# Rose-STL-Lab/spherical-dyffusion

Hardware: AMD Instinct MI355X
Metric: forecast-steps/sec (180x360, 63ch), 25-member ensemble DYffusion sampling, whole job (higher is better)
Workload: dtype f32 tensors; every GEMM-class kernel (1x1 convs, fused MLP, Legendre analysis/synthesis, dhconv) as 3-pass split-f16 MFMA with f32 accumulation; FFT / norms / pointwise in f32 (statistics f64)

## Files before the change

### include/sdy_amd.h

```cpp
#ifndef SDY_AMD_H
#define SDY_AMD_H

#include <stddef.h>
#include <stdint.h>

#ifdef __cplusplus
extern "C" {
#endif
#pragma GCC visibility push(default)

#define SDY_OK 0
#define SDY_ERR_ARG (-1)
#define SDY_ERR_UNSUPPORTED (-2)
#define SDY_ERR_ALIGN (-3)
#define SDY_ERR_WORKSPACE (-4)
#define SDY_ERR_NAME (-5)
#define SDY_ERR_SHAPE (-6)
#define SDY_ERR_STATE (-7)

#define SDY_GRID_EQUIANGULAR 0
#define SDY_GRID_LEGENDRE_GAUSS 1

int sdy_version(void);
const char* sdy_error_string(int code);
// ... 30 lines not shown
int sdy_gelu_stats(const float* y, long y_bstride, float* out, long out_bstride, int out_tiled, double* stats, int B, int C,
                   int HW, void* stream);
int sdy_affine_copy_stats(const float* x, long x_bstride, const float* a, const float* d, float* out, long out_bstride,
                          double* stats, int C, int HW, const unsigned char* rows, int n_rows, int src_row0, void* stream);

int sdy_dhconv_pack_weight(const float* w_host, int Ci, int Co, int L, float* w_packed_dev, void* stream);
int sdy_dhconv(const float* Cs_in, const float* w_packed, float* Cs_out, int L, int mtr, int B, int Ci, int Co,
               void* stream);
size_t sdy_dhconv_h3_pack_bytes(int Ci, int Co, int L);
int sdy_dhconv_h3_pack_weight(const float* w_host, int Ci, int Co, int L, void* packed_dev, float* scale);
int sdy_dhconv_h3(const float* Cs_in, const void* packed, float scale, float* Cs_out, int L, int mtr, int B, int Ci,
                  int Co, void* stream);

int sdy_dhconv_frag_supported(int Ci, int Co);
size_t sdy_dhconv_frag_pack_bytes(int L);
int sdy_dhconv_frag_pack(const float* w_host, int L, void* packed_dev, float* scale);
int sdy_dhconv_frag(const float* Cs_in, const void* packed, float scale, float* Cs_out, int L, int mtr, int B,
                    void* stream);

int sdy_instnorm_coeffs(const float* x, int B, int C, int HW, const float* gamma, const float* beta,
                        const float* scale_shift, long ss_stride, float eps, float* a, float* d, void* stream);

typedef struct sdy_conv_args {
  const float* x;  long x_bstride;
  const float* wt; int ldw;
  float* out;      long out_bstride;
  int B, Cin, Cout, HW;
  const float* pa; const float* pd;
  const float* bias;
  const float* add; long add_bstride;
  int add_mode;
  int act;
  float drop_p;
  const float* keep_mask;
  uint64_t seed; uint32_t call; uint32_t stream_id; uint32_t batch_offset;
  int rows_per_call;
  const float* batch_scale;
  int kernel_tag;
  const void* w_h3;
  float w_h3_scale;
  const void* w_frag;
  float w_frag_scale;
  double* stats;
  int out_tiled;
  const unsigned char* x_rows;
} sdy_conv_args;
int sdy_conv1x1(const sdy_conv_args* args, void* stream);

int sdy_conv256_h3_supported(int Cin, int Cout);
size_t sdy_conv256_h3_pack_bytes(void);
size_t sdy_conv256_h3_pack_bytes_cin(int Cin);
int sdy_conv256_h3_pack(const float* w_host, void* packed_dev, float* scale);
int sdy_conv256_h3_pack_cin(const float* w_host, int Cin, void* packed_dev, float* scale);
size_t sdy_h3_pack_bytes(int Cout, int Cin);
int sdy_h3_pack_weight(const float* w_host, int Cout, int Cin, void* packed_dev, float* scale);

typedef struct sdy_mlp_args {
  const float* x;  long x_bstride;
  const float* pa; const float* pd;
  const void* w; float w1_scale; float w2_scale;
  const float* b1; const float* b2;
  float* out;      long out_bstride;
  const float* add; long add_bstride;
  const float* add_a; const float* add_d;
  int B, E, hidden, HW;
  float drop_p;
  uint64_t seed; uint32_t call; uint32_t stream_fc1; uint32_t stream_fc2; uint32_t batch_offset;
  int rows_per_call;
  const float* batch_scale;
  double* stats;
  int x_tiled;
  const float* keep_hidden;
  const float* keep_out;
  const unsigned char* out_rows;
  int add_by_launch_row;
} sdy_mlp_args;
int sdy_instnorm_from_stats(double* stats, int B, int C, int HW, const float* gamma, const float* beta,
                            const float* scale_shift, long ss_bstride, float eps, float* a_out, float* d_out, void* stream);
int sdy_mlp_h3_supported(int E, int hidden);
size_t sdy_mlp_h3_pack_bytes(int E, int hidden);
int sdy_mlp_h3_pack(const float* w1_host, const float* w2_host, int E, int hidden, void* packed_dev, float* scale1,
                    float* scale2);
int sdy_mlp_h3(const sdy_mlp_args* args, void* stream);

typedef struct sdy_pair_args {
  const float* x;  long x_bstride;
  const void* w; float w1_scale; float w2_scale;
  const float* b1;
  float* out;      long out_bstride;
  const float* add; long add_bstride;
  int B, Cin, hidden, Cout, HW;
  double* stats;
} sdy_pair_args;
int sdy_pair_h3_supported(int Cin, int hidden, int Cout);
size_t sdy_pair_h3_pack_bytes(int Cin, int hidden, int Cout);
int sdy_pair_h3_pack(const float* w1_host, const float* w2_host, int Cin, int hidden, int Cout, void* packed_dev,
                     float* scale1, float* scale2);
int sdy_pair_h3(const sdy_pair_args* args, void* stream);

typedef struct sdy_sfno_config {
  int nlat, nlon;
  int in_chans;
  int out_chans;
  int embed_dim;
  int num_layers;
  int mlp_hidden;
// ... 594 lines not shown
```

### spherical-dyffusion_amd/_lib.py

```python
from __future__ import annotations

import ctypes as C
import os

_HERE = os.path.dirname(os.path.abspath(__file__))
LIB_PATH = os.environ.get("SDY_AMD_LIB") or os.path.join(_HERE, "libsdy_amd.so")

SDY_GRID = {"equiangular": 0, "legendre-gauss": 1}


class SdyError(RuntimeError):
    pass


class SdyConvArgs(C.Structure):
    _fields_ = [
        ("x", C.c_void_p), ("x_bstride", C.c_long),
        ("wt", C.c_void_p), ("ldw", C.c_int),
        ("out", C.c_void_p), ("out_bstride", C.c_long),
        ("B", C.c_int), ("Cin", C.c_int), ("Cout", C.c_int), ("HW", C.c_int),
        ("pa", C.c_void_p), ("pd", C.c_void_p),
        ("bias", C.c_void_p),
        ("add", C.c_void_p), ("add_bstride", C.c_long),
        ("add_mode", C.c_int),
# ... 556 lines not shown
    "sdy_sht_tables_host": (C.c_int, [C.c_int, C.c_int, C.c_int, C.c_int, C.c_int, C.c_void_p, C.c_void_p, C.c_void_p]),
    "sdy_sht_plan_create": (C.c_int, [C.c_int, C.c_int, C.c_int, C.c_int, C.c_int, C.POINTER(C.c_void_p)]),
    "sdy_sht_plan_create_ex": (C.c_int, [C.c_int, C.c_int, C.c_int, C.c_int, C.c_int, C.c_int, C.POINTER(C.c_void_p)]),
    "sdy_sht_plan_destroy": (None, [C.c_void_p]),
    "sdy_sht_plan_dims": (C.c_int, [C.c_void_p, C.POINTER(C.c_int * 6)]),
    "sdy_sht_plan_kernels": (C.c_int, [C.c_void_p, C.POINTER(C.c_int * 2)]),
    "sdy_sht_workspace_floats": (C.c_size_t, [C.c_void_p, C.c_int, C.c_int]),
    "sdy_sht_forward": (C.c_int, [C.c_void_p, C.c_void_p, C.c_void_p, C.c_int, C.c_int, C.c_void_p, C.c_size_t, C.c_void_p]),
    "sdy_sht_inverse": (C.c_int, [C.c_void_p, C.c_void_p, C.c_void_p, C.c_int, C.c_int, C.c_void_p, C.c_size_t, C.c_void_p]),
    "sdy_rfft_lon": (C.c_int, [C.c_void_p, C.c_void_p, C.c_void_p, C.c_void_p, C.c_void_p, C.c_void_p, C.c_int, C.c_int, C.c_void_p]),
    "sdy_legendre_fwd": (C.c_int, [C.c_void_p, C.c_void_p, C.c_void_p, C.c_int, C.c_int, C.c_void_p]),
    "sdy_legendre_inv": (C.c_int, [C.c_void_p, C.c_void_p, C.c_void_p, C.c_int, C.c_int, C.c_void_p]),
    "sdy_irfft_lon": (C.c_int, [C.c_void_p, C.c_void_p, C.c_void_p, C.c_void_p, C.c_int, C.c_int, C.c_void_p]),
    "sdy_irfft_lon_act": (C.c_int, [C.c_void_p, C.c_void_p, C.c_void_p, C.c_void_p, C.c_long, C.c_void_p, C.c_int, C.c_int,
                                    C.c_void_p]),
    "sdy_instnorm_from_partials": (C.c_int, [C.c_void_p, C.c_int, C.c_int, C.c_int, C.c_int, C.c_void_p, C.c_void_p, C.c_float,
                                             C.c_void_p, C.c_void_p, C.c_void_p]),
    "sdy_gelu_stats": (C.c_int, [C.c_void_p, C.c_long, C.c_void_p, C.c_long, C.c_int, C.c_void_p, C.c_int, C.c_int, C.c_int,
                                 C.c_void_p]),
    "sdy_affine_copy_stats": (C.c_int, [C.c_void_p, C.c_long, C.c_void_p, C.c_void_p, C.c_void_p, C.c_long, C.c_void_p, C.c_int,
                                        C.c_int, C.c_void_p, C.c_int, C.c_int, C.c_void_p]),
    "sdy_dhconv_pack_weight": (C.c_int, [C.c_void_p, C.c_int, C.c_int, C.c_int, C.c_void_p, C.c_void_p]),
    "sdy_dhconv": (C.c_int, [C.c_void_p, C.c_void_p, C.c_void_p, C.c_int, C.c_int, C.c_int, C.c_int, C.c_int, C.c_void_p]),
    "sdy_dhconv_h3_pack_bytes": (C.c_size_t, [C.c_int, C.c_int, C.c_int]),
    "sdy_dhconv_h3_pack_weight": (C.c_int, [C.c_void_p, C.c_int, C.c_int, C.c_int, C.c_void_p, C.POINTER(C.c_float)]),
    "sdy_dhconv_h3": (C.c_int, [C.c_void_p, C.c_void_p, C.c_float, C.c_void_p, C.c_int, C.c_int, C.c_int, C.c_int, C.c_int,
                                C.c_void_p]),
    "sdy_dhconv_frag_supported": (C.c_int, [C.c_int, C.c_int]),
    "sdy_dhconv_frag_pack_bytes": (C.c_size_t, [C.c_int]),
    "sdy_dhconv_frag_pack": (C.c_int, [C.c_void_p, C.c_int, C.c_void_p, C.POINTER(C.c_float)]),
    "sdy_dhconv_frag": (C.c_int, [C.c_void_p, C.c_void_p, C.c_float, C.c_void_p, C.c_int, C.c_int, C.c_int, C.c_void_p]),
    "sdy_instnorm_coeffs": (C.c_int, [C.c_void_p, C.c_int, C.c_int, C.c_int, C.c_void_p, C.c_void_p, C.c_void_p, C.c_long,
                                      C.c_float, C.c_void_p, C.c_void_p, C.c_void_p]),
    "sdy_conv1x1": (C.c_int, [C.POINTER(SdyConvArgs), C.c_void_p]),
    "sdy_ensemble_metrics": (C.c_int, [C.c_void_p, C.c_void_p, C.c_void_p, C.c_int, C.c_long, C.c_int, C.c_int, C.c_void_p,
                                       C.c_void_p]),
    "sdy_instnorm_from_stats": (C.c_int, [C.c_void_p, C.c_int, C.c_int, C.c_int, C.c_void_p, C.c_void_p, C.c_void_p,
                                          C.c_long, C.c_float, C.c_void_p, C.c_void_p, C.c_void_p]),
    "sdy_mlp_h3_supported": (C.c_int, [C.c_int, C.c_int]),
    "sdy_mlp_h3_pack_bytes": (C.c_size_t, [C.c_int, C.c_int]),
    "sdy_mlp_h3_pack": (C.c_int, [C.c_void_p, C.c_void_p, C.c_int, C.c_int, C.c_void_p, C.POINTER(C.c_float),
                                  C.POINTER(C.c_float)]),
    "sdy_mlp_h3": (C.c_int, [C.POINTER(SdyMlpArgs), C.c_void_p]),
    "sdy_pair_h3_supported": (C.c_int, [C.c_int, C.c_int, C.c_int]),
    "sdy_pair_h3_pack_bytes": (C.c_size_t, [C.c_int, C.c_int, C.c_int]),
    "sdy_pair_h3_pack": (C.c_int, [C.c_void_p, C.c_void_p, C.c_int, C.c_int, C.c_int, C.c_void_p, C.POINTER(C.c_float),
                                   C.POINTER(C.c_float)]),
    "sdy_pair_h3": (C.c_int, [C.POINTER(SdyPairArgs), C.c_void_p]),
    "sdy_conv256_h3_supported": (C.c_int, [C.c_int, C.c_int]),
    "sdy_conv256_h3_pack_bytes": (C.c_size_t, []),
    "sdy_conv256_h3_pack_bytes_cin": (C.c_size_t, [C.c_int]),
    "sdy_conv256_h3_pack": (C.c_int, [C.c_void_p, C.c_void_p, C.POINTER(C.c_float)]),
    "sdy_conv256_h3_pack_cin": (C.c_int, [C.c_void_p, C.c_int, C.c_void_p, C.POINTER(C.c_float)]),
    "sdy_h3_pack_bytes": (C.c_size_t, [C.c_int, C.c_int]),
    "sdy_h3_pack_weight": (C.c_int, [C.c_void_p, C.c_int, C.c_int, C.c_void_p, C.POINTER(C.c_float)]),
    "sdy_sfno_create": (C.c_int, [C.POINTER(SdySfnoConfig), C.POINTER(C.c_void_p)]),
    "sdy_sfno_destroy": (None, [C.c_void_p]),
    "sdy_sfno_set_param": (C.c_int, [C.c_void_p, C.c_char_p, C.c_void_p, C.c_size_t]),
    "sdy_sfno_ready": (C.c_int, [C.c_void_p]),
    "sdy_sfno_missing": (C.c_char_p, [C.c_void_p]),
    "sdy_sfno_workspace_floats": (C.c_size_t, [C.c_void_p, C.c_int]),
    "sdy_sfno_max_batch": (C.c_int, [C.c_void_p]),
    "sdy_sfno_forward": (C.c_int, [C.c_void_p, C.POINTER(SdySfnoFwdArgs), C.c_void_p]),
    "sdy_sfno_time_embed": (C.c_int, [C.c_void_p, C.c_void_p, C.c_int, C.c_void_p, C.c_void_p, C.c_void_p]),
    "sdy_norm_pack": (C.c_int, [C.POINTER(SdyVarTable), C.c_int, C.c_int, C.c_int, C.c_int, C.c_void_p, C.c_void_p]),
    "sdy_step_finish": (C.c_int, [C.POINTER(SdyStepFinishArgs), C.c_void_p]),
    "sdy_init_timeline": (C.c_int, [C.POINTER(SdyVarTable), C.c_int, C.c_int, C.c_int, C.POINTER(C.c_void_p),
                                    C.POINTER(C.c_void_p), C.c_void_p]),
    "sdy_lp_rel_terms": (C.c_int, [C.c_void_p, C.POINTER(SdyVarTable), C.c_int, C.c_int, C.c_int, C.c_int, C.c_void_p,
                                   C.c_void_p]),
    "sdy_cold_update": (C.c_int, [C.c_void_p, C.c_void_p, C.c_void_p, C.c_void_p, C.c_size_t, C.c_void_p]),
    "sdy_concat_channels": (C.c_int, [C.POINTER(C.c_void_p), C.POINTER(C.c_int), C.c_int, C.c_void_p, C.c_int, C.c_int,
                                      C.c_void_p]),
    "sdy_time_mean_accumulate": (C.c_int, [C.c_void_p, C.c_int, C.c_long, C.c_int, C.c_long, C.c_int, C.c_int, C.c_int,
                                          C.c_float, C.c_void_p, C.c_void_p]),
    "sdy_status_flags": (C.c_int, [C.POINTER(C.c_uint), C.c_int, C.c_void_p]),
    "sdy_status_flags_async": (C.c_int, [C.c_void_p, C.c_int, C.c_void_p]),
    "sdy_range_headroom_enable": (C.c_int, [C.c_int]),
    "sdy_range_headroom": (C.c_int, [C.POINTER(C.c_float), C.c_int, C.c_void_p]),
    "sdy_dropout_stream_rounds": (C.c_int, []),
    "sdy_dropout_stream_words": (C.c_int, [C.c_uint32, C.c_uint32, C.c_uint32, C.c_uint32, C.c_uint32, C.c_uint32,
                                           C.POINTER(C.c_uint32)]),
    "sdy_cond_noise_fill": (C.c_int, [C.c_uint64, C.c_uint32, C.c_uint32, C.c_int, C.c_int, C.c_int, C.c_int, C.c_void_p,
                                      C.c_void_p]),
    "sdy_ensemble_series": (C.c_int, [C.c_void_p, C.c_int, C.c_long, C.c_long, C.c_void_p, C.c_long, C.c_void_p, C.c_int,
                                     C.c_int, C.c_int, C.c_void_p, C.c_void_p]),
    "sdy_ensemble_series_grad": (C.c_int, [C.c_void_p, C.c_int, C.c_long, C.c_long, C.c_void_p, C.c_long, C.c_void_p,
                                          C.c_int, C.c_int, C.c_int, C.c_int, C.c_void_p, C.c_void_p]),
    "sdy_derived_water": (C.c_int, [C.POINTER(SdyDerivedArgs), C.c_void_p]),
    "sdy_corrector": (C.c_int, [C.POINTER(SdyCorrectorArgs), C.c_void_p]),
    "sdy_corrector_host": (C.c_int, [C.POINTER(SdyCorrectorArgs)]),
    "sdy_corrector_workspace_bytes": (C.c_size_t, [C.c_int, C.c_int]),
    "sdy_dry_air_series": (C.c_int, [C.POINTER(SdyDryAirArgs), C.c_void_p]),
    "sdy_dry_air_series_host": (C.c_int, [C.POINTER(SdyDryAirArgs)]),
    "sdy_dry_air_workspace_bytes": (C.c_size_t, [C.c_int, C.c_int, C.c_int]),
    "sdy_hist_add": (C.c_int, [C.POINTER(SdyHistArgs), C.c_void_p]),
    "sdy_hist_state_bytes": (C.c_size_t, [C.c_int]),
    "sdy_hist_state_unpack_host": (C.c_int, [C.c_void_p, C.c_int, C.POINTER(C.c_float), C.POINTER(C.c_float),
                                             C.POINTER(C.c_int), C.POINTER(C.c_uint), C.POINTER(C.c_ulonglong)]),
    "sdy_hist_plan_host": (C.c_int, [C.c_float, C.c_float, C.c_int, C.c_float, C.c_float, C.c_int, C.POINTER(C.c_float),
                                     C.POINTER(C.c_float), C.POINTER(C.c_int), C.POINTER(C.c_int), C.POINTER(C.c_uint)]),
    "sdy_hist_edges_host": (C.c_int, [C.c_float, C.c_float, C.c_int, C.c_void_p]),
    "sdy_hist_bins_host": (C.c_int, [C.c_void_p, C.c_long, C.c_float, C.c_float, C.c_int, C.c_void_p]),
    "sdy_time_coarsen": (C.c_int, [C.POINTER(SdyCoarsenArgs), C.c_void_p]),
    "sdy_time_coarsen_host": (C.c_int, [C.POINTER(SdyCoarsenArgs)]),
    "sdy_video_accumulate": (C.c_int, [C.POINTER(SdyVideoArgs), C.c_void_p]),
# ... 128 lines not shown
```

### spherical-dyffusion_amd/csrc/common.h

```cpp
#pragma once
#include <hip/hip_runtime.h>
#include <stdint.h>
#include <atomic>
#include <cmath>
#include <type_traits>

#include "../../include/sdy_amd.h"

#define SDY_HIP_TRY(expr)                       \
  do {                                          \
    hipError_t _e = (expr);                     \
    if (_e != hipSuccess) return (int)_e;       \
  } while (0)

#define SDY_TRY(expr)             \
  do {                            \
    int _r = (expr);              \
    if (_r != SDY_OK) return _r;  \
  } while (0)

static inline int sdy_launch_status() {
  hipError_t e = hipGetLastError();
  return e == hipSuccess ? SDY_OK : (int)e;
}
// ... 105 lines not shown
    const unsigned bits = __float_as_uint(amax);
    if (bits > *reinterpret_cast<volatile unsigned*>(head)) atomicMax(head, bits);
  }
}
#ifdef SDY_NT_STORE
#define SDY_STREAM_STORE(ptr, v) __builtin_nontemporal_store((v), reinterpret_cast<f32x4*>(ptr))
#else
#define SDY_STREAM_STORE(ptr, v) (*reinterpret_cast<f32x4*>(ptr) = (v))
#endif
typedef float f32x16 __attribute__((ext_vector_type(16)));
__device__ __forceinline__ float sdy_quad_sum(f32x4 v) { return (v.x + v.y) + (v.z + v.w); }
__device__ __forceinline__ float sdy_quad_sumsq(f32x4 v) {
  return __builtin_fmaf(v.x, v.x, v.y * v.y) + __builtin_fmaf(v.z, v.z, v.w * v.w);
}
__device__ __forceinline__ float row16_sum(float x) {
  auto dpp = [](float v, auto ctrl) {
    return __builtin_bit_cast(float, __builtin_amdgcn_update_dpp(0, __builtin_bit_cast(int, v), decltype(ctrl)::value, 0xF, 0xF, true));
  };
  x += dpp(x, std::integral_constant<int, 0xB1>{});
  x += dpp(x, std::integral_constant<int, 0x4E>{});
  x += dpp(x, std::integral_constant<int, 0x141>{});
  x += dpp(x, std::integral_constant<int, 0x140>{});
  return x;
}

#ifdef SDY_STAMPS
#define SDY_STAMPS_ON 1
#else
#define SDY_STAMPS_ON 0
#endif
#define SDY_DEBUG_EXPORT extern "C" __attribute__((visibility("default")))

#ifndef SDY_H3_PASSES
#define SDY_H3_PASSES 3
#endif
#define SDY_CROSS_TERM(stmt) do { if (SDY_H3_PASSES == 3) { stmt; } } while (0)

typedef const char __attribute__((address_space(1)))* sdy_gcptr_t;
typedef char __attribute__((address_space(1)))* sdy_gptr_t;
typedef f32x4 __attribute__((address_space(1))) sdy_gf32x4;
__device__ __forceinline__ f32x4 sdy_ld16s(const float* ubase, unsigned off_b) {
  sdy_gcptr_t b = (sdy_gcptr_t)ubase;
  asm volatile("" : "+s"(b), "+v"(off_b));
  return *reinterpret_cast<const sdy_gf32x4*>(b + off_b);
}
__device__ __forceinline__ void sdy_st16s(float* ubase, unsigned off_b, f32x4 v) {
  sdy_gptr_t b = (sdy_gptr_t)ubase;
  asm volatile("" : "+s"(b), "+v"(off_b));
#ifdef SDY_NT_STORE
  __builtin_nontemporal_store(v, reinterpret_cast<sdy_gf32x4*>(b + off_b));
#else
  *reinterpret_cast<sdy_gf32x4*>(b + off_b) = v;
#endif
}

__device__ __forceinline__ sdy_f16x8 sdy_ring_ld(const void* ubase, unsigned& off, int imm) {
  sdy_gcptr_t b = (sdy_gcptr_t)ubase;
  asm volatile("" : "+s"(b), "+v"(off));
  return *reinterpret_cast<const sdy_f16x8 __attribute__((address_space(1)))*>(b + off + imm);
}

__device__ __forceinline__ float gelu_erf(float x) {
  const float z = fabsf(x) * 0.70710678118654752440f;
  const float t = __builtin_amdgcn_rcpf(fmaf(0.3275911f, z, 1.0f));
  float q = fmaf(1.061405429f, t, -1.453152027f);
  q = fmaf(q, t, 1.421413741f);
  q = fmaf(q, t, -0.284496736f);
  q = fmaf(q, t, 0.254829592f);
  q = q * t * __builtin_amdgcn_exp2f(-z * z * 1.44269504088896340736f);
  const float hq = 0.5f * q;
  return x >= 0.0f ? x * (1.0f - hq) : x * hq;
}
typedef float sdy_gf2 __attribute__((ext_vector_type(2)));
__device__ __forceinline__ sdy_gf2 gelu_erf2(sdy_gf2 x) {
  const sdy_gf2 ax = __builtin_elementwise_abs(x);
  const sdy_gf2 z = ax * 0.70710678118654752440f;
  const sdy_gf2 d = z * 0.3275911f + 1.0f;
  const sdy_gf2 t = {__builtin_amdgcn_rcpf(d.x), __builtin_amdgcn_rcpf(d.y)};
  sdy_gf2 q = t * 1.061405429f + -1.453152027f;
  q = q * t + 1.421413741f;
  q = q * t + -0.284496736f;
  q = q * t + 0.254829592f;
  const sdy_gf2 e2 = z * z * -1.44269504088896340736f;
  const sdy_gf2 e = {__builtin_amdgcn_exp2f(e2.x), __builtin_amdgcn_exp2f(e2.y)};
  const sdy_gf2 hq = q * t * e * 0.5f;
  const sdy_gf2 pos = x * (1.0f - hq), neg = x * hq;
  return sdy_gf2{x.x >= 0.0f ? pos.x : neg.x, x.y >= 0.0f ? pos.y : neg.y};
}
#define SDY_GELU_NODES 385
#define SDY_GELU_TAB_BYTES (SDY_GELU_NODES * 16)
#define SDY_GELU_SX SDY_ACT_SX
#define SDY_GELU_WS 8.0f
#define SDY_GELU_MAGIC (8388608.0f + 192.0f)
int sdy_gelu_table_ptr(const float** table_dev);
typedef const f32x4 __attribute__((address_space(3)))* sdy_lds_f32x4_cptr;
__device__ __forceinline__ f32x4 gelu_tab_load(unsigned addr) { return *reinterpret_cast<sdy_lds_f32x4_cptr>((uintptr_t)addr); }
__device__ __forceinline__ float gelu_tab16(float w, unsigned tab_lds_base) {
  const float wc = __builtin_amdgcn_fmed3f(w, -6.0f * SDY_GELU_WS, 6.0f * SDY_GELU_WS);
  const float t = fmaf(wc, 4.0f, SDY_GELU_MAGIC);
  const f32x4 c = gelu_tab_load((__builtin_bit_cast(unsigned, t) << 4) + (tab_lds_base - 0xB0000000u));
  const float f = fmaf(wc, 4.0f, -(t - SDY_GELU_MAGIC));
  return w * fmaf(fmaf(fmaf(c.w, f, c.z), f, c.y), f, c.x);
}
__device__ __forceinline__ void gelu_tab_to_lds(float* dst, const float* tab_global, int tid, int nthreads, float scale = 1.0f) {
  for (int i = tid; i < SDY_GELU_NODES; i += nthreads)
    reinterpret_cast<f32x4*>(dst)[i] = reinterpret_cast<const f32x4*>(tab_global)[i] * scale;
// ... 108 lines not shown
```

### spherical-dyffusion_amd/csrc/conv_h3.hip

```cpp
#include <cmath>
#include <cstdlib>
#include <type_traits>
#include <vector>

#include "common.h"

namespace {

constexpr int CE = 256;
constexpr int CTN = 64;
constexpr int CKMAX = 384;
constexpr int CRING = 4;
constexpr float CSX = SDY_ACT_SX;
constexpr int CSTAT_BYTES = CE * 2 * 8;
#ifndef SDY_CONV_STAMP_T0
#define SDY_CONV_STAMP_T0 2
#endif

template <int KBLK, int NW>
struct ConvCfg {
  static_assert(NW == 4 || NW == 8, "4 or 8 waves");
  static constexpr int NT = 64 * NW;
  static constexpr int MT = 8 / NW;
  static constexpr int RS = 4 * NW;
  static constexpr int OC = (8 * KBLK + RS - 1) / RS;
  static constexpr int RPT = 64 / NW;
  static constexpr int PPI = (8 * OC + RPT - 1) / RPT;
  static constexpr int KROW = KBLK <= 4 ? 256 : 384;
  static constexpr int KSW = KROW / 16;
  static constexpr int GPK = 4 * MT;
  static constexpr int GPW = MT * KSW;
  static constexpr int WGS = NW == 4 ? 2 : 1;
  static constexpr int TILE_BYTES = 2 * CTN * KROW * 2;
  static constexpr int LDS_BYTES = TILE_BYTES + CSTAT_BYTES + CE * 4 + SDY_GELU_TAB_BYTES;
};
#ifndef SDY_CONV_GELU_TAB
#define SDY_CONV_GELU_TAB 1
#endif

struct ConvParams {
  const float* x; long x_bs;
  const float* pa; const float* pd;
  const sdy_f16x8* w;
  const float* bias;
  const float* add; long add_bs; int add_mode;
  int act;
  float* out; long out_bs;
  int out_tiled;
  double* stats;
  int HW, B;
  int Cin;
  float out_scale;
  unsigned* flags;
  unsigned* head;
  const float* gelu_tab;
  SdyImgMap xmap;
  unsigned long long* stamps;
};

__device__ __forceinline__ int cv_swz(int px) { return (px & 15) ^ (((px >> 4) & 1) * 3); }
template <int KROW>
__device__ __forceinline__ int cv_off(int px, int c) { return px * KROW + (((c & ~15) | ((c ^ cv_swz(px)) & 15)) << 3); }

template <int KBLK, int NW, bool WS = false>
__global__ __launch_bounds__(64 * NW, NW == 4 ? 2 : 1) void conv_h3_kernel(const ConvParams p) {
  using G = ConvCfg<KBLK, NW>;
  static_assert(!WS || (KBLK == 4 && NW == 8), "weight-stationary: 256 input channels on 8 waves");
  constexpr int RING = WS ? G::KSW : CRING;
  constexpr int CMT = G::MT, CRS = G::RS, COC = G::OC, CRPT = G::RPT, KROW = G::KROW, CGPK = G::GPK, CGPW = G::GPW;
  __shared__ __attribute__((aligned(16))) unsigned char smem[G::LDS_BYTES];
  _Float16* Xs_hi = reinterpret_cast<_Float16*>(smem);
  _Float16* Xs_lo = Xs_hi + CTN * KROW;
  float* Os = reinterpret_cast<float*>(smem);

  const int tid = threadIdx.x, lane = tid & 63, wave = tid >> 6;
  auto Cin = [&] { return WS ? CE : p.Cin; };
  auto add_mode = [&] { return WS ? 1 : p.add_mode; };
  auto act = [&] { return WS ? 1 : p.act; };
  int h = lane >> 5, l31 = lane & 31;
  int q0 = tid & 15, o0 = tid >> 4;
  const int tpi = (p.HW + CTN - 1) / CTN;
  const int ntiles = tpi * p.B;
  const int t_per = (ntiles + (int)gridDim.x - 1) / (int)gridDim.x;
  const int t_begin = (int)blockIdx.x * t_per;
  const int t_end = (t_begin + t_per < ntiles) ? t_begin + t_per : ntiles;

  sdy_f16x8 r_hi[RING], r_lo[RING];
  constexpr int CGROUP_BYTES = SDY_GROUP * (int)sizeof(sdy_f16x8);
  const int uwave = __builtin_amdgcn_readfirstlane(wave);
  const char* const wbase = reinterpret_cast<const char*>(p.w) +
                            (WS ? (size_t)((uwave >> 1) * 2 * G::KSW + (uwave & 1)) * CGROUP_BYTES : (size_t)uwave * CGPW * CGROUP_BYTES);
  unsigned woff = (unsigned)lane * 16u;
#pragma unroll
  for (int s = 0; s < RING; ++s) {
    r_hi[s] = sdy_ring_ld(wbase, woff, 0);
    r_lo[s] = sdy_ring_ld(wbase, woff, CGROUP_BYTES / 2);
    woff += (WS ? 2 : 1) * CGROUP_BYTES;
  }
  constexpr int NWIN = KBLK * CMT;
  if (!WS && NWIN == 1) woff -= CRING * CGROUP_BYTES;

  double* Ss = reinterpret_cast<double*>(smem + G::TILE_BYTES);
  float* Bs = reinterpret_cast<float*>(smem + G::TILE_BYTES + CSTAT_BYTES);
  if (tid < CE) {
    Bs[tid] = p.bias ? p.bias[tid] / p.out_scale : 0.0f;
    Ss[2 * tid] = 0.0; Ss[2 * tid + 1] = 0.0;
  }
  float* Gt = reinterpret_cast<float*>(smem + G::TILE_BYTES + CSTAT_BYTES + CE * 4);
  const unsigned gt_base = (unsigned)(uintptr_t)Gt;
  const bool tab_gelu = SDY_CONV_GELU_TAB && act() == 1;
  if (tab_gelu) gelu_tab_to_lds(Gt, p.gelu_tab, tid, G::NT, 1.0f / SDY_GELU_SX);
  const float os_scale = tab_gelu ? p.out_scale * SDY_GELU_WS : p.out_scale;

  f32x4 xr[COC][8], addv[CRPT];
  auto img = [&](const float* base, long bs, int t) { return base + (long)(t / tpi) * bs; };
  auto ximg = [&](int t) { return p.x + (long)sdy_img(p.xmap, t / tpi) * p.x_bs; };
  auto lane_col = [&](int t) {
    const int nn = (t % tpi) * CTN + 4 * q0;
    return nn < p.HW ? nn : 0;
  };
  const float* addsrc = p.add ? p.add : p.out;
  const long addsrc_bs = p.add ? p.add_bs : p.out_bs;
  if (t_begin < t_end) {
    const float* xz = ximg(t_begin);
    const unsigned xo = (unsigned)(8 * o0 * p.HW + lane_col(t_begin)) * 4u;
#pragma unroll
    for (int oc = 0; oc < COC; ++oc)
#pragma unroll
      for (int e = 0; e < 8; ++e) {
        const int ch = 8 * (o0 + CRS * oc) + e;
        xr[oc][e] = f32x4{0.f, 0.f, 0.f, 0.f};
        if (WS || ch < Cin()) xr[oc][e] = sdy_ld16s(xz + (long)(8 * CRS * oc + e) * p.HW, xo);
      }
  }

  for (int tile = t_begin; tile < t_end; ++tile) {
    asm volatile("" : "+v"(l31), "+v"(h), "+v"(q0), "+v"(o0));
    const int tile_it = tile - t_begin;
    auto stamp = [&](int i) {
      if (SDY_STAMPS_ON && p.stamps && blockIdx.x == 3 && tid == 0 && tile_it >= SDY_CONV_STAMP_T0 && tile_it < SDY_CONV_STAMP_T0 + 4)
        p.stamps[(tile_it - SDY_CONV_STAMP_T0) * 8 + i] = __builtin_amdgcn_s_memtime();
    };
    stamp(0);
    const int z = tile / tpi;
    const int zx = sdy_img(p.xmap, z);
    const int n0 = (tile - z * tpi) * CTN;
    const bool full = n0 + CTN <= p.HW;

    {
      float amax = 0.0f;
      const bool ok = full || (n0 + 4 * q0 < p.HW);
#pragma unroll
      for (int oc = 0; oc < COC; ++oc) {
        const int c0 = 8 * (o0 + CRS * oc);
        if (8 * CRS * oc + 8 * CRS > KROW && c0 >= KROW) continue;
        float av[8], dv[8];
        if (p.pa) {
          const f32x4 a0 = *reinterpret_cast<const f32x4*>(p.pa + (long)zx * CE + c0);
          const f32x4 a1 = *reinterpret_cast<const f32x4*>(p.pa + (long)zx * CE + c0 + 4);
          const f32x4 d0 = *reinterpret_cast<const f32x4*>(p.pd + (long)zx * CE + c0);
          const f32x4 d1 = *reinterpret_cast<const f32x4*>(p.pd + (long)zx * CE + c0 + 4);
#pragma unroll
          for (int e = 0; e < 4; ++e) {
            av[e] = a0[e] * CSX; av[e + 4] = a1[e] * CSX;
            dv[e] = d0[e] * CSX; dv[e + 4] = d1[e] * CSX;
          }
        } else {
#pragma unroll
          for (int e = 0; e < 8; ++e) { av[e] = CSX; dv[e] = 0.f; }
        }
#pragma unroll
        for (int pp = 0; pp < 4; ++pp) {
          sdy_f16x8 vh, vl;
          float v[8];
#pragma unroll
          for (int e = 0; e < 8; ++e) v[e] = (ok && (WS || c0 + e < Cin())) ? fmaf(xr[oc][e][pp], av[e], dv[e]) : 0.0f;
          sdy_split8(v, vh, vl, amax);
          const int off = cv_off<KROW>(4 * q0 + pp, o0 + CRS * oc);
          *reinterpret_cast<sdy_f16x8*>(Xs_hi + off) = vh;
          *reinterpret_cast<sdy_f16x8*>(Xs_lo + off) = vl;
        }
      }
      sdy_flag_range(p.flags, amax, p.head);
    }
    __syncthreads();
    stamp(1);
    const int col = n0 + 4 * q0;
    const bool c_ok = full || col < p.HW;
    const unsigned ro = (unsigned)(o0 * p.HW + (c_ok ? col : 0)) * 4u;
    const unsigned ro_out = p.out_tiled ? (unsigned)(o0 * CTN + 4 * q0) * 4u : ro;
    const int out_rs = p.out_tiled ? CTN : p.HW;
    const int tnext = (tile + 1 < t_end) ? tile + 1 : tile;
    const float* xz_next = ximg(tnext);
    const unsigned xo_next = (unsigned)(8 * o0 * p.HW + lane_col(tnext)) * 4u;
    if constexpr (WS) {
      const float* az = img(p.add, p.add_bs, tile);
#pragma unroll
      for (int i = 0; i < CRPT; ++i) addv[i] = sdy_ld16s(az + (long)(CRS * i) * p.HW, ro);
      __builtin_amdgcn_sched_barrier(0);
    }
    stamp(2);
    f32x16 acc[CMT][2];
#pragma unroll
    for (int mi = 0; mi < CMT; ++mi)
#pragma unroll
      for (int r4 = 0; r4 < 4; ++r4) {
        const f32x4 b4 = *reinterpret_cast<const f32x4*>(Bs + 32 * (CMT * wave + mi) + 8 * r4 + 4 * h);
#pragma unroll
        for (int j = 0; j < 2; ++j)
#pragma unroll
          for (int r = 0; r < 4; ++r) acc[mi][j][4 * r4 + r] = b4[r];
      }
    auto ld_b = [&](int ks, sdy_f16x8* bh, sdy_f16x8* bl) {
#pragma unroll
      for (int j = 0; j < 2; ++j) {
        const int off = cv_off<KROW>(32 * j + l31, 2 * ks + h);
        bh[j] = *reinterpret_cast<const sdy_f16x8*>(Xs_hi + off);
        bl[j] = *reinterpret_cast<const sdy_f16x8*>(Xs_lo + off);
      }
    };
    if constexpr (WS) {
      sdy_f16x8 bh[2][2], bl[2][2];
      ld_b(0, bh[0], bl[0]);
      sdy_static_for<0, G::KSW>([&](auto ks_c) {
        constexpr int ks = decltype(ks_c)::value, c = ks & 1;
        if constexpr (ks + 1 < G::KSW) ld_b(ks + 1, bh[c ^ 1], bl[c ^ 1]);
#pragma unroll
        for (int j = 0; j < 2; ++j) SDY_CROSS_TERM(acc[0][j] = __builtin_amdgcn_mfma_f32_32x32x16_f16(r_lo[ks], bh[c][j], acc[0][j], 0, 0, 0));
#pragma unroll
        for (int j = 0; j < 2; ++j) SDY_CROSS_TERM(acc[0][j] = __builtin_amdgcn_mfma_f32_32x32x16_f16(r_hi[ks], bl[c][j], acc[0][j], 0, 0, 0));
#pragma unroll
        for (int j = 0; j < 2; ++j) acc[0][j] = __builtin_amdgcn_mfma_f32_32x32x16_f16(r_hi[ks], bh[c][j], acc[0][j], 0, 0, 0);
        __builtin_amdgcn_sched_barrier(0);
      });
    } else {
#pragma unroll
    for (int kb = 0; kb < KBLK; ++kb) {
#pragma unroll
      for (int i = 0; i < 4; ++i) {
        const int ks = 4 * kb + i;
        sdy_f16x8 bh[2], bl[2];
        ld_b(ks, bh, bl);
#pragma unroll
        for (int mi = 0; mi < CMT; ++mi) {
          const int g = kb * CGPK + CMT * i + mi;
          const int s = g % CRING;
#pragma unroll
          for (int j = 0; j < 2; ++j) SDY_CROSS_TERM(acc[mi][j] = __builtin_amdgcn_mfma_f32_32x32x16_f16(r_lo[s], bh[j], acc[mi][j], 0, 0, 0));
#pragma unroll
          for (int j = 0; j < 2; ++j) SDY_CROSS_TERM(acc[mi][j] = __builtin_amdgcn_mfma_f32_32x32x16_f16(r_hi[s], bl[j], acc[mi][j], 0, 0, 0));
#pragma unroll
          for (int j = 0; j < 2; ++j) acc[mi][j] = __builtin_amdgcn_mfma_f32_32x32x16_f16(r_hi[s], bh[j], acc[mi][j], 0, 0, 0);
          r_hi[s] = sdy_ring_ld(wbase, woff, 0);
          r_lo[s] = sdy_ring_ld(wbase, woff, CGROUP_BYTES / 2);
          woff += CGROUP_BYTES;
          if ((g + CRING + 1) % (NWIN * CRING) == 0) woff -= NWIN * CRING * CGROUP_BYTES;
          __builtin_amdgcn_sched_barrier(0);
        }
      }
    }
    }

    stamp(3);
    if constexpr (WS) {
      static_assert(!WS || COC == 1, "one channel octet per thread");
#pragma unroll
      for (int e = 0; e < 8; ++e) xr[0][e] = sdy_ld16s(xz_next + (long)e * p.HW, xo_next);
      __builtin_amdgcn_sched_barrier(0);
    } else {
      const float* az = img(addsrc, addsrc_bs, tile);
#pragma unroll
      for (int i = 0; i < CRPT; ++i) addv[i] = p.add ? sdy_ld16s(az + (long)(CRS * i) * p.HW, ro) : f32x4{0.f, 0.f, 0.f, 0.f};
    }
    __syncthreads();
    stamp(4);
#pragma unroll
    for (int mi = 0; mi < CMT; ++mi)
#pragma unroll
      for (int j = 0; j < 2; ++j)
#pragma unroll
        for (int r = 0; r < 16; ++r) {
          const int row = 32 * (CMT * wave + mi) + (r & 3) + 8 * (r >> 2) + 4 * h;
          Os[row * CTN + 32 * j + l31] = acc[mi][j][r] * os_scale;
        }
    __syncthreads();
    stamp(5);
    {
      float* oz = p.out + (long)z * p.out_bs + (p.out_tiled ? (long)(tile - z * tpi) * (CE * CTN) : 0L);
#pragma unroll
      for (int i = 0; i < CRPT; ++i) {
        f32x4 v = *reinterpret_cast<const f32x4*>(Os + (o0 + CRS * i) * CTN + 4 * q0);
        if (tab_gelu) {
          if (add_mode() == 1) v = addv[i] * SDY_GELU_WS + v;
          v = f32x4{gelu_tab16(v.x, gt_base), gelu_tab16(v.y, gt_base), gelu_tab16(v.z, gt_base), gelu_tab16(v.w, gt_base)};
        } else {
        if (add_mode() == 1) v += addv[i];
        if (act() == 1) {
          const sdy_gf2 g0 = gelu_erf2(sdy_gf2{v.x, v.y}), g1 = gelu_erf2(sdy_gf2{v.z, v.w});
          v = f32x4{g0.x, g0.y, g1.x, g1.y};
        }
        }
        if (add_mode() == 2) v += addv[i];
        if (c_ok) sdy_st16s(oz + (long)(CRS * i) * out_rs, ro_out, v);
#pragma unroll
        for (int k = 0; k < G::PPI; ++k) {
          const int piece = G::PPI * i + k, oc = piece >> 3, e = piece & 7;
          if (oc < COC) {
            const int ch = 8 * (o0 + CRS * oc) + e;
            if constexpr (!WS)
              if (ch < Cin()) xr[oc][e] = sdy_ld16s(xz_next + (long)(8 * CRS * oc + e) * p.HW, xo_next);
          }
        }
        if (p.stats) {
          const float s1 = row16_sum(c_ok ? sdy_quad_sum(v) : 0.0f);
          const float s2 = row16_sum(c_ok ? sdy_quad_sumsq(v) : 0.0f);
          if (q0 == 0) {
            double* st = Ss + 2 * (o0 + CRS * i);
            __hip_atomic_fetch_add(st, (double)s1, __ATOMIC_RELAXED, __HIP_MEMORY_SCOPE_WORKGROUP);
            __hip_atomic_fetch_add(st + 1, (double)s2, __ATOMIC_RELAXED, __HIP_MEMORY_SCOPE_WORKGROUP);
          }
        }
      }
    }
    stamp(6);
    {
      const int nt = tile + 1;
      if (p.stats && (nt >= t_end || nt / tpi != z)) {
        __syncthreads();
        if (tid < CE) {
          double* st = p.stats + ((long)z * CE + tid) * 2;
          __hip_atomic_fetch_add(st, Ss[2 * tid], __ATOMIC_RELAXED, __HIP_MEMORY_SCOPE_AGENT);
          __hip_atomic_fetch_add(st + 1, Ss[2 * tid + 1], __ATOMIC_RELAXED, __HIP_MEMORY_SCOPE_AGENT);
          Ss[2 * tid] = 0.0; Ss[2 * tid + 1] = 0.0;
        }
      }
    }
    stamp(7);
    __syncthreads();
  }
}

}

#if SDY_STAMPS_ON
static unsigned long long* g_cstamps = nullptr;
SDY_DEBUG_EXPORT int sdy_conv256_h3_debug_stamps(unsigned long long* host64) {
  if (!g_cstamps || !host64) return SDY_ERR_STATE;
  SDY_HIP_TRY(hipDeviceSynchronize());
  SDY_HIP_TRY(hipMemcpy(host64, g_cstamps, 64 * sizeof(unsigned long long), hipMemcpyDeviceToHost));
  return SDY_OK;
}
#endif

extern "C" int sdy_conv256_h3_supported(int Cin, int Cout) { return (Cin >= 1 && Cin <= CKMAX && Cout == CE) ? 1 : 0; }

static void conv_layout(int Cin, int* nw, int* ksw, int* mt) {
  const int kblk = (Cin + 63) / 64;
  *nw = kblk <= 4 ? 4 : 8;
  *ksw = kblk <= 4 ? 16 : 24;
  *mt = 8 / *nw;
}

extern "C" size_t sdy_conv256_h3_pack_bytes_cin(int Cin) {
  int nw, ksw, mt;
  conv_layout(Cin < 1 ? 1 : Cin, &nw, &ksw, &mt);
  return (size_t)nw * mt * ksw * SDY_GROUP * sizeof(sdy_f16x8);
}
extern "C" size_t sdy_conv256_h3_pack_bytes(void) { return sdy_conv256_h3_pack_bytes_cin(CE); }

extern "C" int sdy_conv256_h3_pack_cin(const float* w_host, int Cin, void* dev, float* scale) {
  if (!w_host || !dev || !scale || Cin < 1 || Cin > CKMAX) return SDY_ERR_ARG;
  const float s = sdy_h3_scale(sdy_h3_absmax(w_host, (size_t)CE * Cin));
  int nw, ksw, mt;
  conv_layout(Cin, &nw, &ksw, &mt);
  const size_t gh = (size_t)SDY_GROUP * 8;
  std::vector<_Float16> buf((size_t)nw * mt * ksw * gh);
  _Float16* d = buf.data();
  for (int w = 0; w < nw; ++w)
    for (int ks = 0; ks < ksw; ++ks)
      for (int mi = 0; mi < mt; ++mi, d += gh)
        sdy_h3_put_group(d, s, [&](int r, int k) {
          const int kk = 16 * ks + k;
          return kk < Cin ? w_host[(size_t)(32 * (mt * w + mi) + r) * Cin + kk] : 0.0f;
        });
  SDY_HIP_TRY(hipMemcpy(dev, buf.data(), buf.size() * sizeof(_Float16), hipMemcpyHostToDevice));
  *scale = s;
  return SDY_OK;
}
extern "C" int sdy_conv256_h3_pack(const float* w_host, void* dev, float* scale) {
  return sdy_conv256_h3_pack_cin(w_host, CE, dev, scale);
}

template <int KBLK, int NW, bool WS = false>
static void conv_launch(const ConvParams& p, long ntiles, int n_cu, hipStream_t stream) {
  using G = ConvCfg<KBLK, NW>;
  const long want = (long)n_cu * G::WGS;
  dim3 grid((unsigned)(ntiles < want ? ntiles : want));
  hipLaunchKernelGGL((conv_h3_kernel<KBLK, NW, WS>), grid, dim3(G::NT), 0, stream, p);
}

int sdy_conv256_h3_ws_form(const sdy_conv_args* a) {
  return a && SDY_CONV_GELU_TAB && a->Cin == CE && a->Cout == CE && a->add_mode == 1 && a->add && a->act == 1;
}

int sdy_conv256_h3_launch(const sdy_conv_args* a, hipStream_t stream, int ws) {
// ... 45 lines not shown
```

Before: 166.9.

## Stage weight-stationary conv residual loads into LDS via global_load_lds DMA

In the weight-stationary 256-channel conv kernel, the residual/add tensor is now loaded with global_load_lds_dwordx4 directly into a dedicated LDS zone instead of into registers. It is read back from LDS in the epilogue, and the next tile's input prefetch moves earlier. Barriers become explicit lgkmcnt waits plus s_barrier, with a partial vmcnt wait before the epilogue. This aims to free VGPRs and overlap the add-tensor fetch with the MFMA main loop, at the cost of 64KB extra LDS (which can lower occupancy) and hand-written m0/waitcnt handling that is fragile. A host mapping helper is exported for verification.

New measurement: 165.7. Within noise of the previous version (-0.7%).

```diff
diff --git a/include/sdy_amd.h b/include/sdy_amd.h
--- a/include/sdy_amd.h
+++ b/include/sdy_amd.h
@@ -106,6 +106,7 @@
 size_t sdy_conv256_h3_pack_bytes_cin(int Cin);
 int sdy_conv256_h3_pack(const float* w_host, void* packed_dev, float* scale);
 int sdy_conv256_h3_pack_cin(const float* w_host, int Cin, void* packed_dev, float* scale);
+int sdy_conv_ws_dma_map_host(int HW, int tile, long long* src_elem, unsigned* dst_lds, unsigned* read_lds, unsigned* base_lds);
 size_t sdy_h3_pack_bytes(int Cout, int Cin);
 int sdy_h3_pack_weight(const float* w_host, int Cout, int Cin, void* packed_dev, float* scale);
 
diff --git a/spherical-dyffusion_amd/_lib.py b/spherical-dyffusion_amd/_lib.py
--- a/spherical-dyffusion_amd/_lib.py
+++ b/spherical-dyffusion_amd/_lib.py
@@ -632,6 +632,7 @@
     "sdy_conv256_h3_pack_bytes_cin": (C.c_size_t, [C.c_int]),
     "sdy_conv256_h3_pack": (C.c_int, [C.c_void_p, C.c_void_p, C.POINTER(C.c_float)]),
     "sdy_conv256_h3_pack_cin": (C.c_int, [C.c_void_p, C.c_int, C.c_void_p, C.POINTER(C.c_float)]),
+    "sdy_conv_ws_dma_map_host": (C.c_int, [C.c_int, C.c_int, C.c_void_p, C.c_void_p, C.c_void_p, C.c_void_p]),
     "sdy_h3_pack_bytes": (C.c_size_t, [C.c_int, C.c_int]),
     "sdy_h3_pack_weight": (C.c_int, [C.c_void_p, C.c_int, C.c_int, C.c_void_p, C.POINTER(C.c_float)]),
     "sdy_sfno_create": (C.c_int, [C.POINTER(SdySfnoConfig), C.POINTER(C.c_void_p)]),
diff --git a/spherical-dyffusion_amd/csrc/common.h b/spherical-dyffusion_amd/csrc/common.h
--- a/spherical-dyffusion_amd/csrc/common.h
+++ b/spherical-dyffusion_amd/csrc/common.h
@@ -181,6 +181,12 @@
 #else
   *reinterpret_cast<sdy_gf32x4*>(b + off_b) = v;
 #endif
+}
+__device__ __forceinline__ void sdy_dma16s(const float* ubase, unsigned off_b, unsigned lds_ubase) {
+  sdy_gcptr_t b = (sdy_gcptr_t)ubase;
+  unsigned keep;
+  asm volatile("s_nop 4\n\ts_mov_b32 %0, m0\n\ts_mov_b32 m0, %3\n\ts_nop 0\n\tglobal_load_lds_dwordx4 %1, %2\n\ts_mov_b32 m0, %0"
+               : "=&s"(keep) : "v"(off_b), "s"(b), "s"(lds_ubase) : "memory");
 }
 
 __device__ __forceinline__ sdy_f16x8 sdy_ring_ld(const void* ubase, unsigned& off, int imm) {
diff --git a/spherical-dyffusion_amd/csrc/conv_h3.hip b/spherical-dyffusion_amd/csrc/conv_h3.hip
--- a/spherical-dyffusion_amd/csrc/conv_h3.hip
+++ b/spherical-dyffusion_amd/csrc/conv_h3.hip
@@ -4,6 +4,7 @@
 #include <vector>
 
 #include "common.h"
+#include "conv_ws_dma.h"
 
 namespace {
 
@@ -68,10 +69,16 @@
   static_assert(!WS || (KBLK == 4 && NW == 8), "weight-stationary: 256 input channels on 8 waves");
   constexpr int RING = WS ? G::KSW : CRING;
   constexpr int CMT = G::MT, CRS = G::RS, COC = G::OC, CRPT = G::RPT, KROW = G::KROW, CGPK = G::GPK, CGPW = G::GPW;
-  __shared__ __attribute__((aligned(16))) unsigned char smem[G::LDS_BYTES];
+  constexpr int ZONE_BYTES = WS ? SDY_CVWS_ZONE_BYTES : 0;
+  static_assert(G::LDS_BYTES + ZONE_BYTES <= 160 * 1024, "one CU's LDS");
+  __shared__ __attribute__((aligned(16))) unsigned char smem_all[G::LDS_BYTES + ZONE_BYTES];
+  unsigned char* const smem = smem_all + ZONE_BYTES;
   _Float16* Xs_hi = reinterpret_cast<_Float16*>(smem);
   _Float16* Xs_lo = Xs_hi + CTN * KROW;
   float* Os = reinterpret_cast<float*>(smem);
+  unsigned char* const amem = smem_all;
+  const unsigned amem_base = (unsigned)(uintptr_t)amem;
+  static_assert(!WS || (G::RS == SDY_CVWS_ROW_STEP && G::RPT == SDY_CVWS_PIECES && CE == SDY_CVWS_ROWS && CTN == SDY_CVWS_PX), "conv_ws_dma.h");
 
   const int tid = threadIdx.x, lane = tid & 63, wave = tid >> 6;
   auto Cin = [&] { return WS ? CE : p.Cin; };
@@ -85,6 +92,15 @@
   const int t_begin = (int)blockIdx.x * t_per;
   const int t_end = (t_begin + t_per < ntiles) ? t_begin + t_per : ntiles;
 
+  auto bar = [&] {
+    if constexpr (WS) {
+      asm volatile("s_waitcnt lgkmcnt(0)" ::: "memory");
+      __builtin_amdgcn_s_barrier();
+      asm volatile("" ::: "memory");
+    } else {
+      __syncthreads();
+    }
+  };
   sdy_f16x8 r_hi[RING], r_lo[RING];
   constexpr int CGROUP_BYTES = SDY_GROUP * (int)sizeof(sdy_f16x8);
   const int uwave = __builtin_amdgcn_readfirstlane(wave);
@@ -183,11 +199,11 @@
       }
       sdy_flag_range(p.flags, amax, p.head);
     }
-    __syncthreads();
+    bar();
     stamp(1);
     const int col = n0 + 4 * q0;
     const bool c_ok = full || col < p.HW;
-    const unsigned ro = (unsigned)(o0 * p.HW + (c_ok ? col : 0)) * 4u;
+    const unsigned ro = WS ? sdy_cvws_lane_off(o0, q0, n0, p.HW) : (unsigned)(o0 * p.HW + (c_ok ? col : 0)) * 4u;
     const unsigned ro_out = p.out_tiled ? (unsigned)(o0 * CTN + 4 * q0) * 4u : ro;
     const int out_rs = p.out_tiled ? CTN : p.HW;
     const int tnext = (tile + 1 < t_end) ? tile + 1 : tile;
@@ -196,7 +212,10 @@
     if constexpr (WS) {
       const float* az = img(p.add, p.add_bs, tile);
 #pragma unroll
-      for (int i = 0; i < CRPT; ++i) addv[i] = sdy_ld16s(az + (long)(CRS * i) * p.HW, ro);
+      for (int i = 0; i < CRPT; ++i) sdy_dma16s(az + sdy_cvws_piece_elem(i, p.HW), ro, amem_base + sdy_cvws_piece_lds(uwave, i));
+      static_assert(!WS || COC == 1, "one channel octet per thread");
+#pragma unroll
+      for (int e = 0; e < 8; ++e) xr[0][e] = sdy_ld16s(xz_next + (long)e * p.HW, xo_next);
       __builtin_amdgcn_sched_barrier(0);
     }
     stamp(2);
@@ -262,17 +281,12 @@
     }
 
     stamp(3);
-    if constexpr (WS) {
-      static_assert(!WS || COC == 1, "one channel octet per thread");
-#pragma unroll
-      for (int e = 0; e < 8; ++e) xr[0][e] = sdy_ld16s(xz_next + (long)e * p.HW, xo_next);
-      __builtin_amdgcn_sched_barrier(0);
-    } else {
+    if constexpr (!WS) {
       const float* az = img(addsrc, addsrc_bs, tile);
 #pragma unroll
       for (int i = 0; i < CRPT; ++i) addv[i] = p.add ? sdy_ld16s(az + (long)(CRS * i) * p.HW, ro) : f32x4{0.f, 0.f, 0.f, 0.f};
     }
-    __syncthreads();
+    bar();
     stamp(4);
 #pragma unroll
     for (int mi = 0; mi < CMT; ++mi)
@@ -283,13 +297,15 @@
           const int row = 32 * (CMT * wave + mi) + (r & 3) + 8 * (r >> 2) + 4 * h;
           Os[row * CTN + 32 * j + l31] = acc[mi][j][r] * os_scale;
         }
-    __syncthreads();
+    if constexpr (WS) asm volatile("s_waitcnt vmcnt(8)" ::: "memory");
+    bar();
     stamp(5);
     {
       float* oz = p.out + (long)z * p.out_bs + (p.out_tiled ? (long)(tile - z * tpi) * (CE * CTN) : 0L);
 #pragma unroll
       for (int i = 0; i < CRPT; ++i) {
         f32x4 v = *reinterpret_cast<const f32x4*>(Os + (o0 + CRS * i) * CTN + 4 * q0);
+        if constexpr (WS) addv[i] = *reinterpret_cast<const f32x4*>(amem + sdy_cvws_read_lds(o0, q0, i));
         if (tab_gelu) {
           if (add_mode() == 1) v = addv[i] * SDY_GELU_WS + v;
           v = f32x4{gelu_tab16(v.x, gt_base), gelu_tab16(v.y, gt_base), gelu_tab16(v.z, gt_base), gelu_tab16(v.w, gt_base)};
@@ -326,7 +342,7 @@
     {
       const int nt = tile + 1;
       if (p.stats && (nt >= t_end || nt / tpi != z)) {
-        __syncthreads();
+        bar();
         if (tid < CE) {
           double* st = p.stats + ((long)z * CE + tid) * 2;
           __hip_atomic_fetch_add(st, Ss[2 * tid], __ATOMIC_RELAXED, __HIP_MEMORY_SCOPE_AGENT);
@@ -336,7 +352,7 @@
       }
     }
     stamp(7);
-    __syncthreads();
+    bar();
   }
 }
 
@@ -351,6 +367,22 @@
   return SDY_OK;
 }
 #endif
+
+extern "C" int sdy_conv_ws_dma_map_host(int HW, int tile, long long* src_elem, unsigned* dst_lds, unsigned* read_lds, unsigned* base_lds) {
+  if (!src_elem || !dst_lds || !read_lds || !base_lds || HW <= 0 || (HW & 3) || tile < 0 || (long)tile * CTN >= HW) return SDY_ERR_ARG;
+  const int n0 = tile * CTN;
+  for (int w = 0; w < SDY_CVWS_WAVES; ++w)
+    for (int i = 0; i < SDY_CVWS_PIECES; ++i) {
+      base_lds[w * SDY_CVWS_PIECES + i] = sdy_cvws_piece_lds(w, i);
+      for (int l = 0; l < 64; ++l) {
+        const int k = (w * SDY_CVWS_PIECES + i) * 64 + l, o0 = sdy_cvws_o0(w, l), q0 = sdy_cvws_q0(l);
+        src_elem[k] = (long long)sdy_cvws_piece_elem(i, HW) + (long long)(sdy_cvws_lane_off(o0, q0, n0, HW) / 4u);
+        dst_lds[k] = sdy_cvws_piece_lds(w, i) + 16u * (unsigned)l;
+        read_lds[k] = sdy_cvws_read_lds(o0, q0, i);
+      }
+    }
+  return SDY_OK;
+}
 
 extern "C" int sdy_conv256_h3_supported(int Cin, int Cout) { return (Cin >= 1 && Cin <= CKMAX && Cout == CE) ? 1 : 0; }
 
diff --git a/spherical-dyffusion_amd/csrc/conv_ws_dma.h b/spherical-dyffusion_amd/csrc/conv_ws_dma.h
--- /dev/null
+++ b/spherical-dyffusion_amd/csrc/conv_ws_dma.h
@@ -0,0 +1,29 @@
+#pragma once
+
+#if defined(__HIPCC__) || defined(__CUDACC__)
+#define SDY_CVWS_HD __host__ __device__ inline
+#else
+#define SDY_CVWS_HD inline
+#endif
+
+constexpr int SDY_CVWS_ROWS = 256;
+constexpr int SDY_CVWS_PX = 64;
+constexpr int SDY_CVWS_WAVES = 8;
+constexpr int SDY_CVWS_PIECES = 8;
+constexpr int SDY_CVWS_ROW_STEP = 32;
+constexpr int SDY_CVWS_ZONE_BYTES = SDY_CVWS_ROWS * SDY_CVWS_PX * 4;
+
+SDY_CVWS_HD int sdy_cvws_o0(int wave, int lane) { return 4 * wave + (lane >> 4); }
+SDY_CVWS_HD int sdy_cvws_q0(int lane) { return lane & 15; }
+
+SDY_CVWS_HD unsigned sdy_cvws_lane_off(int o0, int q0, int n0, int HW) {
+  const int col = n0 + 4 * q0;
+  return (unsigned)(o0 * HW + (col < HW ? col : 0)) * 4u;
+}
+SDY_CVWS_HD long sdy_cvws_piece_elem(int piece, int HW) { return (long)(SDY_CVWS_ROW_STEP * piece) * HW; }
+SDY_CVWS_HD unsigned sdy_cvws_piece_lds(int wave, int piece) {
+  return (unsigned)(4 * wave + SDY_CVWS_ROW_STEP * piece) * (unsigned)(SDY_CVWS_PX * 4);
+}
+SDY_CVWS_HD unsigned sdy_cvws_read_lds(int o0, int q0, int step) {
+  return (unsigned)((o0 + SDY_CVWS_ROW_STEP * step) * SDY_CVWS_PX + 4 * q0) * 4u;
+}
```
